# YaoChengTang/DecNet

Hardware: AMD Instinct MI355X
Metric: stereo pairs/sec at 960x540x192disp (hot path: stage-0 dense + SpaMat/SpaVar stages 1-3) (higher is better)
Workload: dtype f32 (bf16x3 on the bf16 matrix pipe); 1 GPU; BASELINE config 2: synthetic 960x540 (padded 972x540), max_disp 192->216: batch=8 synthetic pairs per GPU, feature maps of the 4-stage/scale-3 net, random-init CostRegNetNoDown(216); pairs_per_gpu=8, parallelism=dp1 (pairs sharded, all_gather of disparity maps)

## Files before the change

### decnet_amd/csrc/spamat_mfma.hip

```cpp
#include <stdlib.h>
#include <string.h>

#include "spamat_host.h"


typedef float f32x4 __attribute__((ext_vector_type(4)));
typedef int i32x4 __attribute__((ext_vector_type(4)));
typedef __bf16 bf16x8 __attribute__((ext_vector_type(8)));

namespace {

constexpr float NEG_BIG = -1.0e30f;
constexpr float LOG2E = 1.4426950408889634f;
constexpr int THREADS = 512, NWAVE = THREADS / 64;

__device__ __forceinline__ float fast_exp2(float x) { return __builtin_amdgcn_exp2f(x); }

__device__ __forceinline__ bool uniform_flag(bool f) { return __builtin_amdgcn_readfirstlane((int)f) != 0; }
template <bool SEL = true>
__device__ __forceinline__ float4 load4f(const float *__restrict__ safe, const float *__restrict__ row, int x, int W, bool ok) {
    const bool in = ok && x >= 0 && x < W;
    const float4 t = *reinterpret_cast<const float4 *>(in ? row + x : safe);
    if (!SEL) return t;
    return make_float4(in ? t.x : 0.f, in ? t.y : 0.f, in ? t.z : 0.f, in ? t.w : 0.f);
// ... 7 lines not shown
        if (x + 1 >= 0 && x + 1 < W) v.y = row[x + 1];
        if (x + 2 >= 0 && x + 2 < W) v.z = row[x + 2];
        if (x + 3 >= 0 && x + 3 < W) v.w = row[x + 3];
    }
    return v;
}
__device__ __forceinline__ float4 load4s(const float *__restrict__ row, int x, int W) {
    float4 v = make_float4(0.f, 0.f, 0.f, 0.f);
    if (x >= 0 && x < W) v.x = row[x];
    if (x + 1 >= 0 && x + 1 < W) v.y = row[x + 1];
    if (x + 2 >= 0 && x + 2 < W) v.z = row[x + 2];
    if (x + 3 >= 0 && x + 3 < W) v.w = row[x + 3];
    return v;
}

__device__ __forceinline__ int mask4_bits(const unsigned long long *__restrict__ rowbits, int x, int W) {
    if (x < 0 || x >= W) return 0;
    return (int)((rowbits[x >> 6] >> (x & 63)) & 15ull);
}

__device__ __forceinline__ int mask4_words(const unsigned *__restrict__ roww, int x, int W) {
    if (x < 0 || x >= W) return 0;
    return (int)((roww[x >> 5] >> (x & 31)) & 15u);
}

__device__ __forceinline__ void split3x8(const float (&x)[8], i32x4 &hi, i32x4 &mid, i32x4 &lo) {
    int h[8], m[8], l[8];
#pragma unroll
    for (int e = 0; e < 8; ++e) {
        h[e] = __float_as_int(x[e]) & 0xffff0000;
        const float r1 = x[e] - __int_as_float(h[e]);
        m[e] = __float_as_int(r1) & 0xffff0000;
        l[e] = __float_as_int(r1 - __int_as_float(m[e]));
    }
#pragma unroll
    for (int e = 0; e < 4; ++e) {
        hi[e] = __builtin_amdgcn_perm(h[2 * e + 1], h[2 * e], 0x07060302);
        mid[e] = __builtin_amdgcn_perm(m[2 * e + 1], m[2 * e], 0x07060302);
        lo[e] = __builtin_amdgcn_perm(l[2 * e + 1], l[2 * e], 0x07060302);
    }
}

__host__ __device__ inline int d16_pitch(int quads) { return quads + ((4 - quads) & 7); }
struct Layout {
    int SW, HALO, RP, Cq;
    int offR, offBX, offRK, offLM, offXL, offWT, total;
};
__host__ __device__ inline Layout make_layout(int C, int NT, int XT, bool d16 = false) {
    Layout l;
    l.SW = XT * 16;
    l.HALO = (NT - 1) * 16;
    l.Cq = (C + 3) & ~3;
    l.RP = ((l.HALO + l.SW + 31) & ~31) + 16;
    l.offR = 0;
    const int swh = ((XT + 1) / 2) * 16;
    const int rt = d16 ? 3 * ((C + 7) / 8) * 16 * (d16_pitch((l.HALO + swh) >> 2) + d16_pitch(swh >> 2)) : 0;
    l.offBX = l.offR + (l.Cq * l.RP > rt ? l.Cq * l.RP : rt);
    l.offRK = l.offBX + l.RP;
    l.offLM = l.offRK + l.RP + 4;
    l.offXL = l.offLM + l.SW + 16;
    l.offWT = l.offXL + l.SW;
    l.total = l.offWT + 32;
    return l;
}

__device__ __forceinline__ int wave_incl_scan(int v, int lane) {
#pragma unroll
    for (int o = 1; o < 64; o <<= 1) {
        int t = __shfl_up(v, o);
        if (lane >= o) v += t;
    }
    return v;
}

template <int M, int N, int STEP, class F>
__device__ __forceinline__ void live_tiles(int ntile, F &&f) {
    if constexpr (M < N) {
        if (STEP > 0 && M >= ntile) return;
        f(std::integral_constant<int, M>{});
        if constexpr (STEP == 2 && M + 1 < N) f(std::integral_constant<int, M + 1>{});
        live_tiles<M + (STEP > 1 ? STEP : 1), N, STEP>(ntile, f);
    }
}
template <int NTL, int MODE, int COMPACT>
__device__ __forceinline__ void softmax_passes(f32x4 (&acc)[NTL], int ntile, int D, int dl,
                                               const float *__restrict__ lds, int bias_off, int xr_off,
                                               int xlj, float mu_in,
                                               float &mx_o, float &S_o, float &mu_o, float &var_o,
                                               int m_lo = 0, int m_hi = 0) {
    constexpr int GS = COMPACT >= 2 ? 2 : COMPACT;
    int dlv = dl;
    asm volatile("" : "+v"(dlv));
    float mx0 = 0.000001f, mx1 = 0.000001f;
    (void)bias_off;
    int xo1 = xr_off;
    asm volatile("" : "+v"(xo1));
    const int *xp1 = reinterpret_cast<const int *>(lds) + xo1;
    const float xlf = (float)xlj, hD = 0.5f * (float)(D - 1), xlh = xlf - hD;
    live_tiles<0, NTL, GS>(ntile, [&](auto mc) {
        constexpr int m = decltype(mc)::value;
        {
            if (COMPACT >= 2) {
                if (COMPACT == 2 || m < m_lo || m >= m_hi) {
                    if (COMPACT == 3) asm volatile("" ::: "memory");
                    const float4 p = *reinterpret_cast<const float4 *>(xp1 + 16 * m);
                    acc[m][0] = fabsf(xlh - p.x) <= hD ? acc[m][0] : NEG_BIG;
                    acc[m][1] = fabsf(xlh - p.y) <= hD ? acc[m][1] : NEG_BIG;
                    acc[m][2] = fabsf(xlh - p.z) <= hD ? acc[m][2] : NEG_BIG;
                    acc[m][3] = fabsf(xlh - p.w) <= hD ? acc[m][3] : NEG_BIG;
                }
            } else if (COMPACT) {
                const int4 p = *reinterpret_cast<const int4 *>(xp1 + 16 * m);
                acc[m][0] = (unsigned)(xlj - p.x) < (unsigned)D ? acc[m][0] : NEG_BIG;
                acc[m][1] = (unsigned)(xlj - p.y) < (unsigned)D ? acc[m][1] : NEG_BIG;
                acc[m][2] = (unsigned)(xlj - p.z) < (unsigned)D ? acc[m][2] : NEG_BIG;
                acc[m][3] = (unsigned)(xlj - p.w) < (unsigned)D ? acc[m][3] : NEG_BIG;
            } else {
                if (m == 0 || 16 * m + 15 >= D) {
                    asm volatile("" ::: "memory");
#pragma unroll
                    for (int r = 0; r < 4; ++r) {
                        const int d = 16 * m + dlv - r;
                        acc[m][r] = (unsigned)d >= (unsigned)D ? NEG_BIG : acc[m][r];
                    }
                }
            }
            mx0 = fmaxf(fmaxf(mx0, acc[m][0]), acc[m][1]);
            mx1 = fmaxf(fmaxf(mx1, acc[m][2]), acc[m][3]);
        }
    });
    float mx = fmaxf(mx0, mx1);
    mx = fmaxf(mx, __shfl_xor(mx, 16));
    mx = fmaxf(mx, __shfl_xor(mx, 32));
    if (!COMPACT && MODE != MODE_MAT) {
        const float nmv = -mx * LOG2E;
        float Sa = 0.f, Sb = 0.f, T16a = 0.f, T16b = 0.f, Tt = 0.f;
#pragma unroll
        for (int m = 0; m < NTL; ++m) {
            if (m < ntile) {
                const float e0 = fast_exp2(fmaf(acc[m][0], LOG2E, nmv));
                const float e1 = fast_exp2(fmaf(acc[m][1], LOG2E, nmv));
                const float e2 = fast_exp2(fmaf(acc[m][2], LOG2E, nmv));
                const float e3 = fast_exp2(fmaf(acc[m][3], LOG2E, nmv));
                const float s4 = (e0 + e1) + (e2 + e3);
                const float t2 = fmaf(6.f, e3, fmaf(4.f, e2, e1 + e1));
                const float qq = fmaf(9.f, e3, fmaf(4.f, e2, e1));
                acc[m][0] = s4;
                acc[m][1] = t2;
                acc[m][2] = qq;
                if (m & 1) { Sb += s4; T16b = fmaf(s4, (float)(16 * m), T16b); }
                else { Sa += s4; T16a = fmaf(s4, (float)(16 * m), T16a); }
                Tt += t2;
            }
        }
        const float dlf = (float)dl;
        float Sl = Sa + Sb;
        float Tl = fmaf(dlf, Sl, fmaf(-0.5f, Tt, T16a + T16b));
        Sl += __shfl_xor(Sl, 16);
        Sl += __shfl_xor(Sl, 32);
        const float S = Sl + 0.000001f;
        float mu = mu_in;
        if (MODE != MODE_VAR) {
            Tl += __shfl_xor(Tl, 16);
            Tl += __shfl_xor(Tl, 32);
            mu = (Tl + 0.000001f) / S;
        }
        const float c0 = dlf - mu;
        float V0 = 0.f, V1 = 0.f;
#pragma unroll
        for (int m = 0; m < NTL; ++m) {
            if (m < ntile) {
                const float A = (float)(16 * m) + c0;
                const float u = fmaf(A, acc[m][0], -acc[m][1]);
                if (m & 1) V1 = fmaf(A, u, V1) + acc[m][2];
                else V0 = fmaf(A, u, V0) + acc[m][2];
            }
        }
        float Vl = V0 + V1;
        Vl += __shfl_xor(Vl, 16);
        Vl += __shfl_xor(Vl, 32);
        mx_o = mx; S_o = S; mu_o = mu; var_o = (Vl + 0.000001f) / S;
        return;
    }
    const float nm = -mx * LOG2E;
    float S0 = 0.f, S1 = 0.f, T0 = 0.f, T1 = 0.f;
    int xo2 = xr_off;
    asm volatile("" : "+v"(xo2));
    const int *xp2 = reinterpret_cast<const int *>(lds) + xo2;
    live_tiles<0, NTL, GS>(ntile, [&](auto mc) {
        constexpr int m = decltype(mc)::value;
        {
            int4 p;
            float4 pf;
            if (COMPACT >= 2) pf = *reinterpret_cast<const float4 *>(xp2 + 16 * m);
            else if (COMPACT) p = *reinterpret_cast<const int4 *>(xp2 + 16 * m);
#pragma unroll
            for (int r = 0; r < 4; r += 2) {
                float e0 = fast_exp2(fmaf(acc[m][r], LOG2E, nm));
                float e1 = fast_exp2(fmaf(acc[m][r + 1], LOG2E, nm));
                acc[m][r] = e0;
                acc[m][r + 1] = e1;
                S0 += e0;
                S1 += e1;
                if (MODE != MODE_VAR) {
                    if (COMPACT >= 2) {
                        T0 = fmaf(e0, xlf - (r == 0 ? pf.x : pf.z), T0);
                        T1 = fmaf(e1, xlf - (r == 0 ? pf.y : pf.w), T1);
                    } else if (COMPACT) {
                        T0 = fmaf(e0, (float)(xlj - (r == 0 ? p.x : p.z)), T0);
                        T1 = fmaf(e1, (float)(xlj - (r == 0 ? p.y : p.w)), T1);
                    } else {
                        T0 = fmaf(e0, (float)(16 * m - r), T0);
                        T1 = fmaf(e1, (float)(16 * m - r - 1), T1);
                    }
                }
            }
        }
    });
    const float dlf = (float)dl;
    float Sl = S0 + S1;
    float Tl = COMPACT ? T0 + T1 : fmaf(dlf, Sl, T0 + T1);
    Sl += __shfl_xor(Sl, 16);
    Sl += __shfl_xor(Sl, 32);
    const float S = Sl + 0.000001f;
    float mu = mu_in;
    if (MODE != MODE_VAR) {
        Tl += __shfl_xor(Tl, 16);
        Tl += __shfl_xor(Tl, 32);
        mu = (Tl + 0.000001f) / S;
    }
    float var = 0.f;
    if (MODE != MODE_MAT) {
        const float c0 = (COMPACT ? (float)xlj : dlf) - mu;
        float V0 = 0.f, V1 = 0.f;
        int xo3 = xr_off;
        asm volatile("" : "+v"(xo3));
        const int *xp3 = reinterpret_cast<const int *>(lds) + xo3;
        live_tiles<0, NTL, GS>(ntile, [&](auto mc) {
            constexpr int m = decltype(mc)::value;
            {
                int4 p;
                float4 pf;
                if (COMPACT >= 2) pf = *reinterpret_cast<const float4 *>(xp3 + 16 * m);
                else if (COMPACT) p = *reinterpret_cast<const int4 *>(xp3 + 16 * m);
#pragma unroll
                for (int r = 0; r < 4; r += 2) {
                    float d0, d1;
                    if (COMPACT >= 2) {
                        d0 = c0 - (r == 0 ? pf.x : pf.z);
                        d1 = c0 - (r == 0 ? pf.y : pf.w);
                    } else if (COMPACT) {
                        d0 = c0 - (float)(r == 0 ? p.x : p.z);
                        d1 = c0 - (float)(r == 0 ? p.y : p.w);
                    } else {
                        d0 = (float)(16 * m - r) + c0;
                        d1 = (float)(16 * m - r - 1) + c0;
                    }
                    V0 = fmaf(acc[m][r] * d0, d0, V0);
                    V1 = fmaf(acc[m][r + 1] * d1, d1, V1);
                }
            }
        });
        float Vl = V0 + V1;
        Vl += __shfl_xor(Vl, 16);
        Vl += __shfl_xor(Vl, 32);
        var = (Vl + 0.000001f) / S;
    }
    mx_o = mx; S_o = S; mu_o = mu; var_o = var;
}


__device__ __forceinline__ void dense16_loads8(float4 (&v)[8], const float *__restrict__ src, size_t plane, int g, int C,
                                               int x, int W, bool al) {
    if (al) {
        const bool whole = x + 3 < W;
#pragma unroll
        for (int c = 0; c < 8; ++c)
            v[c] = load4f<false>(src, src + (size_t)(8 * g + c) * plane, x, W, whole && 8 * g + c < C);
        __builtin_amdgcn_sched_barrier(0);
        if (__ballot(x < 0) != 0ull) {
#pragma unroll
            for (int c = 0; c < 8; ++c)
                if (x < 0) v[c] = make_float4(0.f, 0.f, 0.f, 0.f);
        }
        if (C & 7) {
#pragma unroll
            for (int c = 0; c < 8; ++c) {
                const bool ch = 8 * g + c < C;
                v[c] = make_float4(ch ? v[c].x : 0.f, ch ? v[c].y : 0.f, ch ? v[c].z : 0.f, ch ? v[c].w : 0.f);
            }
        }
        if ((W & 3) && x < W && !whole) {
#pragma unroll
            for (int c = 0; c < 8; ++c)
                v[c] = 8 * g + c < C ? load4s(src + (size_t)(8 * g + c) * plane, x, W) : make_float4(0.f, 0.f, 0.f, 0.f);
        }
    } else {
#pragma unroll
        for (int c = 0; c < 8; ++c)
            v[c] = 8 * g + c < C ? load4s(src + (size_t)(8 * g + c) * plane, x, W) : make_float4(0.f, 0.f, 0.f, 0.f);
    }
}

__device__ __forceinline__ void dense16_item_loads(float4 (&v)[8], int it, const float *__restrict__ lrow,
                                                   const float *__restrict__ rrow, size_t plane, int C, int W, int xs,
                                                   int SW, int HALO, int nRw) {
    const bool al = uniform_flag(((((uintptr_t)rrow) | ((uintptr_t)lrow) | ((uintptr_t)(plane * 4))) & 15) == 0);
    const int cg_n = (C + 7) >> 3, nqR = nRw >> 2, nqL = SW >> 2;
    const int nR_items = cg_n * nqR;
    const bool isL = it >= nR_items;
    const int k = isL ? it - nR_items : it, nq = isL ? nqL : nqR;
    const int g = k / nq, jq = k - g * nq;
    const float *src = isL ? lrow : rrow;
    const int x = isL ? xs + 4 * jq : xs - HALO + 4 * jq;
    dense16_loads8(v, src, plane, g, C, x, W, al);
}

template <int NT, int MODE, int CGT, bool PRE = false>
__device__ __forceinline__ void dense16_body(int *RT, const float *BX, const float *LM, const float *smem,
                                             const float *__restrict__ lrow, const float *__restrict__ rrow,
                                             const float *__restrict__ disparity, float *__restrict__ out,
                                             float *__restrict__ var_out, float *__restrict__ sum_sim,
                                             float *__restrict__ max_cost, size_t plane, size_t rowpix, int C, int W,
                                             int D, int xs, int XT, int SW, int HALO, int nRw, const float4 *pre = nullptr) {
    const int tid = threadIdx.x, lane = tid & 63, wave = tid >> 6;
    struct { int CG; } lo = {(C + 7) >> 3};
    const int PR = d16_pitch(nRw >> 2), PL = d16_pitch(SW >> 2);
    int *LT = RT + 3 * lo.CG * 16 * PR;
    {
        const bool al = uniform_flag(((((uintptr_t)rrow) | ((uintptr_t)lrow) | ((uintptr_t)(plane * 4))) & 15) == 0);
        const int cg_n = lo.CG, nqR = nRw >> 2, nqL = SW >> 2;
        const int nR_items = cg_n * nqR, n_items = nR_items + cg_n * nqL;
#pragma unroll 1
        for (int it = tid; it < n_items; it += THREADS) {
            const bool isL = it >= nR_items;
            const int k = isL ? it - nR_items : it, nq = isL ? nqL : nqR;
            const int g = k / nq, jq = k - g * nq;
            const float *src = isL ? lrow : rrow;
            const int x = isL ? xs + 4 * jq : xs - HALO + 4 * jq;
            float4 v[8];
            if (PRE && it == tid) {
#pragma unroll
                for (int c = 0; c < 8; ++c) v[c] = pre[c];
            } else {
                dense16_loads8(v, src, plane, g, C, x, W, al);
            }
            const int P = isL ? PL : PR;
            int *dst = (isL ? LT : RT) + (g * 4 * P + jq) * 4;
            const int tstride = cg_n * 16 * P;
#pragma unroll
            for (int pz = 0; pz < 4; ++pz) {
                float xv[8];
#pragma unroll
                for (int c = 0; c < 8; ++c) xv[c] = pz == 0 ? v[c].x : pz == 1 ? v[c].y : pz == 2 ? v[c].z : v[c].w;
                i32x4 th, tm, tl;
                split3x8(xv, th, tm, tl);
                *reinterpret_cast<i32x4 *>(dst + pz * 4 * P) = th;
                *reinterpret_cast<i32x4 *>(dst + tstride + pz * 4 * P) = tm;
                *reinterpret_cast<i32x4 *>(dst + 2 * tstride + pz * 4 * P) = tl;
            }
        }
    }
    __syncthreads();

    const int j = lane & 15, q = lane >> 4;
    const int dl = j - 4 * q;
    constexpr int CGB = CGT ? CGT : 1;
    const int cg_n = CGT ? CGT : lo.CG;
    const int tA_big = q >> 1, tA_small = q == 0 ? 0 : q == 2 ? 1 : 2;
    const int tB_big = q & 1, tB_small = q == 1 ? 0 : q == 3 ? 1 : 2;
    const int gsR = 16 * PR, gsL = 16 * PL;
    for (int xt = wave; xt < XT; xt += NWAVE) {
        const int x0 = xs + xt * 16;
        if (x0 >= W) break;
        const int x = x0 + j;
        const size_t pix = rowpix + x;
        const bool inside = x < W;
        const float rm = LM[xt * 16 + j];
        if (__ballot(rm != 0.f) == 0ull) {
            if (inside && q == 0) {
                if (MODE != MODE_VAR) out[pix] = 0.f;
                if (MODE != MODE_MAT) var_out[pix] = 0.f;
                sum_sim[pix] = 0.f;
                max_cost[pix] = 0.f;
            }
            continue;
        }
        f32x4 acc[NT];
#pragma unroll
        for (int m = 0; m < NT; ++m) {
            const float4 bz = *reinterpret_cast<const float4 *>(BX + (HALO + xt * 16) + 4 * q - 16 * m);
            acc[m] = f32x4{bz.x, bz.y, bz.z, bz.w};
        }
        const int sa = (j & 3) * PR + 4 * xt + (j >> 2), sb = (j & 3) * PL + 4 * xt + (j >> 2);
        const int *a_small = RT + (tA_small * cg_n * 4 * PR + sa) * 4;
        const int *a_big = RT + (tA_big * cg_n * 4 * PR + sa) * 4;
        const int *b_small = LT + (tB_small * cg_n * 4 * PL + sb) * 4;
        const int *b_big = LT + (tB_big * cg_n * 4 * PL + sb) * 4;
#pragma unroll
        for (int g = 0; g < CGB; ++g) {
            for (int gg = g; gg < cg_n; gg += CGB) {
                const i32x4 bs = *reinterpret_cast<const i32x4 *>(b_small + gg * gsL);
                const i32x4 bb = *reinterpret_cast<const i32x4 *>(b_big + gg * gsL);
#pragma unroll
                for (int m = 0; m < NT; ++m) {
                    const i32x4 av = *reinterpret_cast<const i32x4 *>(a_small + gg * gsR + (NT - 1 - m) * 16);
                    acc[m] = __builtin_amdgcn_mfma_f32_16x16x32_bf16(__builtin_bit_cast(bf16x8, av),
                                                                     __builtin_bit_cast(bf16x8, bs), acc[m], 0, 0, 0);
                }
#pragma unroll
                for (int m = 0; m < NT; ++m) {
                    const i32x4 av = *reinterpret_cast<const i32x4 *>(a_big + gg * gsR + (NT - 1 - m) * 16);
                    acc[m] = __builtin_amdgcn_mfma_f32_16x16x32_bf16(__builtin_bit_cast(bf16x8, av),
                                                                     __builtin_bit_cast(bf16x8, bb), acc[m], 0, 0, 0);
                }
            }
        }
        float mx, S, mu, var;
        const float mu_in = (MODE == MODE_VAR && inside) ? disparity[pix] : 0.f;
        softmax_passes<NT, MODE, 0>(acc, NT, D, dl, smem, 0, 0, 0, mu_in, mx, S, mu, var);
        if (inside && q == 0) {
            const bool on = rm != 0.f;
            if (MODE != MODE_VAR) out[pix] = on ? mu : 0.f;
            if (MODE != MODE_MAT) var_out[pix] = on ? var : 0.f;
            sum_sim[pix] = on ? S : 0.f;
            max_cost[pix] = on ? mx : 0.f;
        }
    }

}

template <int NT, int MODE, int KQ, int PPT, int NTHR, int CAP, int NTCMAX>
__device__ __forceinline__ int sparse_row_body(
    const float *__restrict__ ref, const float *__restrict__ tar, const float *__restrict__ rmask,
    const float *__restrict__ tmask, const float *__restrict__ disparity, float *__restrict__ out,
    float *__restrict__ var_out, float *__restrict__ sum_sim, float *__restrict__ max_cost, int C,
    int H, int W, int D, int row, int dense_pct, int mbits, int *fr_out = nullptr, int *fl_out = nullptr);
constexpr int MID_CAP = 640;

template <int NT, int MODE, int KQ, bool D16>
__device__ __forceinline__ void spamat_fwd_segment(
    const float *__restrict__ ref, const float *__restrict__ tar, const float *__restrict__ rmask,
    const float *__restrict__ tmask, const float *__restrict__ disparity, float *__restrict__ out,
    float *__restrict__ var_out, float *__restrict__ sum_sim, float *__restrict__ max_cost, int C,
    int H, int W, int D, int XT, int allow_compact, int marker, int seg, int row, int compact_pct, int mbits) {
    const float mark = marker ? sum_sim[(size_t)row * W + (size_t)seg * (XT * 16)] : -1.0f;
    if (marker && !(mark < 0.f))
        return;
    if constexpr (KQ == 2) {
        if (marker == 2 && mark == -2.0f) {
            if (sparse_row_body<NT, MODE, KQ, 4, THREADS, MID_CAP, NT + 1>(ref, tar, rmask, tmask, disparity, out, var_out,
                                                                          sum_sim, max_cost, C, H, W, D, row, 100,
                                                                          mbits) == 1)
                return;
            __syncthreads();
        }
    }
    extern __shared__ __attribute__((aligned(16))) float smem[];
    const Layout lo = make_layout(C, NT, XT, D16);
    float *Rs = smem + lo.offR;
    float *BX = smem + lo.offBX;
    int *XR = reinterpret_cast<int *>(BX);
    int *RK = reinterpret_cast<int *>(smem + lo.offRK);
    float *LM = smem + lo.offLM;
    int *RKL = reinterpret_cast<int *>(LM);
    int *XL = reinterpret_cast<int *>(smem + lo.offXL);
    int *WT = reinterpret_cast<int *>(smem + lo.offWT);
    const int SW = lo.SW, HALO = lo.HALO, RP = lo.RP;
    const int kq_n = KQ ? KQ : lo.Cq / 4;
    constexpr int KB = KQ ? KQ : 1;

    const int tid = threadIdx.x, lane = tid & 63, wave = tid >> 6;
    const int b = row / H, y = row - b * H;
    const int xs = seg * SW;
    const int nRw = HALO + SW;
    const size_t plane = (size_t)H * W;
    const float *lrow = ref + ((size_t)b * C * H + y) * W;
    const float *rrow = tar + ((size_t)b * C * H + y) * W;
    const float *trow = tmask + (size_t)row * W;
    const float *mrow = rmask + (size_t)row * W;
    const size_t rowpix = (size_t)row * W;
    const unsigned long long *tbits = reinterpret_cast<const unsigned long long *>(tmask) + (size_t)row * ((W + 63) >> 6);
    const unsigned long long *lbits = reinterpret_cast<const unsigned long long *>(rmask) + (size_t)row * ((W + 63) >> 6);

    unsigned mf_wr = 0, mf_wl = 0;
    if constexpr (D16) {
        if (mbits == 2) {
            const int q4 = tid * 4, xr_ = xs - HALO + q4, xl_ = xs + q4;
            const unsigned *hw = reinterpret_cast<const unsigned *>(max_cost + rowpix);
            mf_wr = hw[(q4 < nRw && xr_ >= 0 && xr_ < W) ? xr_ >> 5 : 0];
            mf_wl = hw[((W + 31) >> 5) + ((q4 < SW && xl_ < W) ? xl_ >> 5 : 0)];
        }
    }
    float4 d16_pre[D16 ? 8 : 1];
    if constexpr (D16) {
        const int xta = (XT + 1) / 2;
        const int n_items = ((C + 7) >> 3) * (((HALO + xta * 16) >> 2) + ((xta * 16) >> 2));
        if (tid < n_items) dense16_item_loads(d16_pre, tid, lrow, rrow, plane, C, W, xs, xta * 16, HALO, HALO + xta * 16);
    }
    const bool al_r = ((((uintptr_t)rrow) | ((uintptr_t)(plane * 4))) & 15) == 0;
    const int st_nq = nRw >> 2;
    const int st_rpp = THREADS / st_nq;
    const int st_r0 = tid / st_nq, st_jq = tid - st_r0 * st_nq;
    float4 st_v[D16 ? 1 : 8];
    float bfirst[(!D16 && KQ > 0) ? KQ : 1];
    if constexpr (!D16) {
        if (st_r0 < st_rpp) {
            const int x = xs - HALO + 4 * st_jq;
#pragma unroll
            for (int u = 0; u < 8; ++u) {
                const int c = st_r0 + u * st_rpp;
                st_v[u] = c < C ? load4_lanes(rrow + (size_t)c * plane, x, W, al_r) : make_float4(0.f, 0.f, 0.f, 0.f);
            }
        }
        if constexpr (KQ > 0) {
            const int jl = lane & 15, ql = lane >> 4;
            const int x = xs + wave * 16 + jl;
            const bool ok = wave < XT && x < W;
#pragma unroll
            for (int s = 0; s < KQ; ++s) bfirst[s] = (ok && 4 * s + ql < C) ? lrow[(size_t)(4 * s + ql) * plane + x] : 0.f;
        }
    }

    const int p4 = tid * 4;
    int fr = 0, fl = 0;
    {
        const bool alm = (((uintptr_t)trow) & 15) == 0 && (((uintptr_t)mrow) & 15) == 0;
        const bool almu = D16 && uniform_flag(alm && (W & 3) == 0);
        if (p4 < nRw) {
            const int x = xs - HALO + p4;
            if (mbits == 2) {
                if (D16) fr = (x >= 0 && x < W) ? (int)((mf_wr >> (x & 31)) & 15u) : 0;
                else fr = mask4_words(reinterpret_cast<const unsigned *>(max_cost + rowpix), x, W);
            } else if (mbits) {
                fr = mask4_bits(tbits, x, W);
            } else {
                float4 tv = almu ? load4f(trow, trow, x, W, true) : load4_lanes(trow, x, W, alm);
                fr = (tv.x != 0.f) | ((tv.y != 0.f) << 1) | ((tv.z != 0.f) << 2) | ((tv.w != 0.f) << 3);
            }
            float4 bv4;
            bv4.x = (fr & 1) ? 0.f : NEG_BIG;
            bv4.y = (fr & 2) ? 0.f : NEG_BIG;
            bv4.z = (fr & 4) ? 0.f : NEG_BIG;
            bv4.w = (fr & 8) ? 0.f : NEG_BIG;
            *reinterpret_cast<float4 *>(BX + p4) = bv4;
        }
        if (p4 < SW) {
            float4 mv;
            if (mbits) {
                if (D16 && mbits == 2) fl = (xs + p4 < W) ? (int)((mf_wl >> ((xs + p4) & 31)) & 15u) : 0;
                else fl = mbits == 2 ? mask4_words(reinterpret_cast<const unsigned *>(max_cost + rowpix) + ((W + 31) >> 5), xs + p4, W)
                                : mask4_bits(lbits, xs + p4, W);
                mv = make_float4((fl & 1) ? 1.f : 0.f, (fl & 2) ? 1.f : 0.f, (fl & 4) ? 1.f : 0.f, (fl & 8) ? 1.f : 0.f);
            } else {
                mv = almu ? load4f(mrow, mrow, xs + p4, W, true) : load4_lanes(mrow, xs + p4, W, alm);
                fl = (mv.x != 0.f) | ((mv.y != 0.f) << 1) | ((mv.z != 0.f) << 2) | ((mv.w != 0.f) << 3);
            }
            *reinterpret_cast<float4 *>(LM + p4) = mv;
        }
    }
    {
        const int ir = wave_incl_scan(__popc(fr), lane), il = wave_incl_scan(__popc(fl), lane);
        if (lane == 63) { WT[wave] = ir; WT[8 + wave] = il; }
    }

    int nR = 0, nL = 0;
    bool compact = false;
    if constexpr (D16) {
        __syncthreads();
#pragma unroll
        for (int w = 0; w < NWAVE; ++w) { nR += WT[w]; nL += WT[8 + w]; }
        const int validL = min(SW, W - xs);
        const int validR = min(W, xs + SW) - max(0, xs - HALO);
        compact = allow_compact && ((long)nL * nR * 100 < (long)validL * validR * compact_pct);
        if (!compact) {
            const int xta = (XT + 1) / 2, xtb = XT - xta;
            dense16_body<NT, MODE, (KQ + 1) / 2, true>(reinterpret_cast<int *>(Rs), BX, LM, smem, lrow, rrow, disparity, out,
                                                       var_out, sum_sim, max_cost, plane, rowpix, C, W, D, xs, xta, xta * 16,
                                                       HALO, HALO + xta * 16, d16_pre);
            if (xtb > 0 && xs + xta * 16 < W) {
                __syncthreads();
                dense16_body<NT, MODE, (KQ + 1) / 2>(reinterpret_cast<int *>(Rs), BX + xta * 16, LM + xta * 16, smem, lrow,
                                                     rrow, disparity, out, var_out, sum_sim, max_cost, plane, rowpix, C,
                                                     W, D, xs + xta * 16, xtb, xtb * 16, HALO, HALO + xtb * 16);
            }
            return;
        }
    }
    {
        const bool al = al_r;
        const int rpp = st_rpp;
        const int r0 = st_r0, jq = st_jq;
        if (r0 < rpp) {
            const int jj = 4 * jq, x = xs - HALO + jj;
            for (int c0 = r0; c0 < lo.Cq; c0 += 8 * rpp) {
                float4 v[8];
                if (!D16 && c0 == r0) {
#pragma unroll
                    for (int u = 0; u < 8; ++u) v[u] = st_v[D16 ? 0 : u];
                } else {
#pragma unroll
                    for (int u = 0; u < 8; ++u) {
                        const int c = c0 + u * rpp;
                        v[u] = c < C ? load4_lanes(rrow + (size_t)c * plane, x, W, al) : make_float4(0.f, 0.f, 0.f, 0.f);
                    }
                }
#pragma unroll
                for (int u = 0; u < 8; ++u) {
                    const int c = c0 + u * rpp;
                    if (c < lo.Cq) *reinterpret_cast<float4 *>(Rs + c * RP + jj) = v[u];
                }
            }
        }
        for (int c = tid; c < lo.Cq; c += THREADS) Rs[c * RP + RP - 1] = 0.f;
    }
    __syncthreads();

    const int validL = min(SW, W - xs);
    const int validR = min(W, xs + SW) - max(0, xs - HALO);
    if constexpr (!D16) {
#pragma unroll
        for (int w = 0; w < NWAVE; ++w) { nR += WT[w]; nL += WT[8 + w]; }
        compact = allow_compact && ((long)nL * nR * 100 < (long)validL * validR * compact_pct);
    }

    const int j = lane & 15, q = lane >> 4;

    if constexpr (!D16) if (!compact) {
        const int dl = j - 4 * q;
        float bv[KQ <= 6 ? KB : 1], bcur[KB];
        float rm = 0.f;
        auto fetch_left = [&](int xt, float (&dst)[KB]) {
            const int x = xs + xt * 16 + j;
            const bool ok = xt < XT && x < W;
            if (KQ) {
#pragma unroll
                for (int s = 0; s < KQ; ++s)
                    dst[s] = (ok && 4 * s + q < C) ? lrow[(size_t)(4 * s + q) * plane + x] : 0.f;
            }
        };
        constexpr bool PREF = KQ <= 6;
        if constexpr (PREF && KQ > 0) {
#pragma unroll
            for (int s = 0; s < KB; ++s) bv[s] = bfirst[s];
        } else if constexpr (PREF) {
            fetch_left(wave, bv);
        }
        for (int xt = wave; xt < XT; xt += NWAVE) {
            const int x0 = xs + xt * 16;
            if (x0 >= W) break;
            const int x = x0 + j;
            const size_t pix = rowpix + x;
            const bool inside = x < W;
            rm = LM[xt * 16 + j];
            if constexpr (PREF) {
#pragma unroll
                for (int s = 0; s < KB; ++s) bcur[s] = bv[s];
                fetch_left(xt + NWAVE, bv);
            } else if (KQ > 0 && xt == wave) {
#pragma unroll
                for (int s = 0; s < KB; ++s) bcur[s] = bfirst[KQ > 0 ? s : 0];
            } else {
// ... 87 lines not shown
    while (S > 16 && (long)S * nL > 24L * validL) S >>= 1;
    __syncthreads();
    constexpr int NTC = NT + 1;
    while (S > 16) {
        int bad = 0;
        for (int g = tid; g * S < SW; g += THREADS) {
            const int jlo = max(0, g * S + HALO - (D - 1)), jhi = min(nRw - 1, g * S + HALO + S - 1);
            if (RK[jhi + 1] - RK[jlo] > 16 * NTC - 15) bad = 1;
        }
        if (!__syncthreads_or(bad)) break;
        S >>= 1;
    }

    for (int p = tid; p < validL; p += THREADS) {
        if (RKL[p + 1] == RKL[p]) {
            const size_t pix = rowpix + xs + p;
            if (MODE != MODE_VAR) out[pix] = 0.f;
            if (MODE != MODE_MAT) var_out[pix] = 0.f;
            sum_sim[pix] = 0.f;
            max_cost[pix] = 0.f;
        }
    }

    const int ngroups = (SW + S - 1) / S;
    for (int g = wave; g < ngroups; g += NWAVE) {
        const int gx = g * S;
        const int e0 = __builtin_amdgcn_readfirstlane(RKL[gx]), e1 = __builtin_amdgcn_readfirstlane(RKL[min(gx + S, SW)]);
        if (e1 == e0) continue;
        const int jlo = max(0, gx + HALO - (D - 1)), jhi = min(nRw - 1, gx + HALO + S - 1);
        const int r_lo = __builtin_amdgcn_readfirstlane(RK[jlo]), r_hi = __builtin_amdgcn_readfirstlane(RK[jhi + 1]);
        const int t0 = r_lo >> 4;
        const int ntile = r_hi > r_lo ? ((r_hi - 1) >> 4) - t0 + 1 : 0;
        for (int e = e0; e < e1; e += 16) {
            const bool act = e + j < e1;
            const int xl = XL[act ? e + j : e1 - 1];
            const int x = xs + xl;
            const size_t pix = rowpix + x;
            float bcur[KB];
            if (KQ) {
#pragma unroll
                for (int s = 0; s < KQ; ++s)
                    bcur[s] = (act && 4 * s + q < C) ? lrow[(size_t)(4 * s + q) * plane + x] : 0.f;
            }
            f32x4 acc[NTC];
            const int *xa = XR + 16 * t0 + j;
            live_tiles<0, NTC, 1>(ntile, [&](auto mc) {
                constexpr int m = decltype(mc)::value;
                {
                    const float *ap = Rs + q * RP + xa[16 * m];
                    f32x4 a4 = f32x4{0.f, 0.f, 0.f, 0.f};
                    if (KQ) {
#pragma unroll
                        for (int s = 0; s < KQ; ++s)
                            a4 = __builtin_amdgcn_mfma_f32_16x16x4f32(ap[4 * s * RP], bcur[s], a4, 0, 0, 0);
                    } else {
                        const float *bp = lrow + (size_t)q * plane + x;
                        for (int s = 0; s < kq_n; ++s) {
                            const float lv = (act && 4 * s + q < C) ? bp[(size_t)4 * s * plane] : 0.f;
                            a4 = __builtin_amdgcn_mfma_f32_16x16x4f32(ap[4 * s * RP], lv, a4, 0, 0, 0);
                        }
                    }
                    acc[m] = a4;
                }
            });
            float mx, Ssum, mu, var;
            const float mu_in = (MODE == MODE_VAR && act) ? disparity[pix] : 0.f;
            softmax_passes<NTC, MODE, 1>(acc, ntile, D, 0, smem, 0, lo.offBX + 16 * t0 + 4 * q, xl + HALO, mu_in,
                                         mx, Ssum, mu, var);
            if (act && q == 0) {
                if (MODE != MODE_VAR) out[pix] = mu;
                if (MODE != MODE_MAT) var_out[pix] = var;
                sum_sim[pix] = Ssum;
                max_cost[pix] = mx;
            }
        }
    }
}

template <int NT, int MODE, int KQ, bool D16>
__global__ __launch_bounds__(THREADS, (KQ > 6 ? 2 : 4)) void spamat_fwd_mfma(
    const float *__restrict__ ref, const float *__restrict__ tar, const float *__restrict__ rmask,
    const float *__restrict__ tmask, const float *__restrict__ disparity, float *__restrict__ out,
    float *__restrict__ var_out, float *__restrict__ sum_sim, float *__restrict__ max_cost, int C,
    int H, int W, int D, int segs_per_row, int XT, int allow_compact, int marker, int compact_pct, int mbits) {
    spamat_fwd_segment<NT, MODE, KQ, D16>(ref, tar, rmask, tmask, disparity, out, var_out, sum_sim, max_cost, C, H, W,
                                          D, XT, allow_compact, marker, blockIdx.x % segs_per_row,
                                          blockIdx.x / segs_per_row, compact_pct, mbits);
}

constexpr int SP_THREADS = 256, SP_CAP = 256;
constexpr size_t sparse_row_words(int kq, int ppt, int nthr, int cap) {
    return (size_t)(cap + 32) + 2 * (size_t)(nthr * ppt / 2 + 2) + cap + 32 + 2 * (size_t)4 * kq * (cap + 16);
}

template <int NT, int MODE, int KQ, int PPT, int NTHR, int CAP, int NTCMAX>
__device__ __forceinline__ int sparse_row_body(
    const float *__restrict__ ref, const float *__restrict__ tar, const float *__restrict__ rmask,
    const float *__restrict__ tmask, const float *__restrict__ disparity, float *__restrict__ out,
    float *__restrict__ var_out, float *__restrict__ sum_sim, float *__restrict__ max_cost, int C,
    int H, int W, int D, int row, int dense_pct, int mbits, int *fr_out, int *fl_out) {
    constexpr int CQ = 4 * KQ, NTC = NT + 1 < NTCMAX ? NT + 1 : NTCMAX;
    constexpr int SP_NWAVE_ = NTHR / 64, SP_FP_ = CAP + 16;
    extern __shared__ __attribute__((aligned(16))) float smem[];
    constexpr int NPX = NTHR * PPT, RKW = NPX / 2 + 2;
    constexpr int offXR = 0, offRK = CAP + 32, offRKL = offRK + RKW, offXL = offRKL + RKW,
                  offWT = offXL + CAP, offRF = offWT + 32, offLF = offRF + CQ * SP_FP_;
    float *XR = smem + offXR;
    unsigned short *RK = reinterpret_cast<unsigned short *>(smem + offRK);
    unsigned short *RKL = reinterpret_cast<unsigned short *>(smem + offRKL);
    int *XL = reinterpret_cast<int *>(smem) + offXL;
    int *WT = reinterpret_cast<int *>(smem) + offWT;
    float *RF = smem + offRF, *LF = smem + offLF;

    const int tid = threadIdx.x, lane = tid & 63, wave = tid >> 6;
    const int b = row / H, y = row - b * H;
    const size_t plane = (size_t)H * W, rowpix = (size_t)row * W;
    const float *lrow = ref + ((size_t)b * C * H + y) * W;
    const float *rrow = tar + ((size_t)b * C * H + y) * W;
    const float *trow = tmask + rowpix, *mrow = rmask + rowpix;

    constexpr bool ALL = CAP > 256 && PPT == 4;
    const int p4 = tid * PPT;
    float4 lv[ALL ? CQ : 1], rv[ALL ? CQ : 1];
    if constexpr (ALL) {
        const bool alf = ((W & 3) == 0) && ((((uintptr_t)lrow) | ((uintptr_t)rrow) | ((uintptr_t)(plane * 4))) & 15) == 0;
#pragma unroll
        for (int c = 0; c < CQ; ++c) {
            const bool ok = p4 < W && c < C;
            lv[c] = ok ? load4_lanes(lrow + (size_t)c * plane, p4, W, alf) : make_float4(0.f, 0.f, 0.f, 0.f);
            rv[c] = ok ? load4_lanes(rrow + (size_t)c * plane, p4, W, alf) : make_float4(0.f, 0.f, 0.f, 0.f);
        }
    }
    int fr = 0, fl = 0;
    {
        const bool alm = ((W & 3) == 0) && ((((uintptr_t)trow) | ((uintptr_t)mrow)) & 15) == 0;
#pragma unroll
        for (int u = 0; u < PPT; u += 4) {
            if (p4 + u < W) {
                if (mbits == 2) {
                    const unsigned *hw = reinterpret_cast<const unsigned *>(max_cost + rowpix);
                    fr |= mask4_words(hw, p4 + u, W) << u;
                    fl |= mask4_words(hw + ((W + 31) >> 5), p4 + u, W) << u;
                } else if (mbits) {
                    const int wpr = (W + 63) >> 6;
                    fr |= mask4_bits(reinterpret_cast<const unsigned long long *>(tmask) + (size_t)row * wpr, p4 + u, W) << u;
                    fl |= mask4_bits(reinterpret_cast<const unsigned long long *>(rmask) + (size_t)row * wpr, p4 + u, W) << u;
                } else {
                    const float4 tv = load4_lanes(trow, p4 + u, W, alm), mv = load4_lanes(mrow, p4 + u, W, alm);
                    fr |= ((tv.x != 0.f) | ((tv.y != 0.f) << 1) | ((tv.z != 0.f) << 2) | ((tv.w != 0.f) << 3)) << u;
                    fl |= ((mv.x != 0.f) | ((mv.y != 0.f) << 1) | ((mv.z != 0.f) << 2) | ((mv.w != 0.f) << 3)) << u;
                }
            }
        }
    }
    if (fr_out) { *fr_out = fr; *fl_out = fl; }
    const int cr = __popc(fr), cl = __popc(fl);
    const int ir = wave_incl_scan(cr, lane), il = wave_incl_scan(cl, lane);
    if (lane == 63) { WT[wave] = ir; WT[8 + wave] = il; }
    __syncthreads();
    int nR = 0, nL = 0, baseR = 0, baseL = 0;
#pragma unroll
    for (int w = 0; w < SP_NWAVE_; ++w) {
        if (w < wave) { baseR += WT[w]; baseL += WT[8 + w]; }
        nR += WT[w];
        nL += WT[8 + w];
    }
    nR = __builtin_amdgcn_readfirstlane(nR);
    nL = __builtin_amdgcn_readfirstlane(nL);
    if ((long)nL * nR * 100 >= (long)W * W * dense_pct) return 0;
    if (nL > CAP || nR > CAP) return (nL <= MID_CAP && nR <= MID_CAP) ? 2 : 0;
// ... 137 lines not shown
                if (MODE != MODE_VAR) *reinterpret_cast<float4 *>(out + pix) = make_float4(r[0][0], r[0][1], r[0][2], r[0][3]);
                if (MODE != MODE_MAT) *reinterpret_cast<float4 *>(var_out + pix) = make_float4(r[1][0], r[1][1], r[1][2], r[1][3]);
                *reinterpret_cast<float4 *>(sum_sim + pix) = make_float4(r[2][0], r[2][1], r[2][2], r[2][3]);
                *reinterpret_cast<float4 *>(max_cost + pix) = make_float4(r[3][0], r[3][1], r[3][2], r[3][3]);
            } else {
#pragma unroll
                for (int k = 0; k < 4; ++k) {
                    if (p4 + u + k < W) {
                        if (MODE != MODE_VAR) out[pix + k] = r[0][k];
                        if (MODE != MODE_MAT) var_out[pix + k] = r[1][k];
                        sum_sim[pix + k] = r[2][k];
                        max_cost[pix + k] = r[3][k];
                    }
                }
            }
        }
    }
    return 1;
}

template <int NT, int MODE, int KQ, int PPT>
__global__ __launch_bounds__(SP_THREADS, PPT == 4 ? 6 : 5) void spamat_fwd_sparse(
    const float *__restrict__ ref, const float *__restrict__ tar, const float *__restrict__ rmask,
    const float *__restrict__ tmask, const float *__restrict__ disparity, float *__restrict__ out,
    float *__restrict__ var_out, float *__restrict__ sum_sim, float *__restrict__ max_cost, int C,
    int H, int W, int D, int seg_w, int dense_pct, int mbits, int handover) {
    const int row = blockIdx.x;
    int fr = 0, fl = 0;
    const int rc = sparse_row_body<NT, MODE, KQ, PPT, SP_THREADS, SP_CAP, 8>(ref, tar, rmask, tmask, disparity, out, var_out,
                                                                            sum_sim, max_cost, C, H, W, D, row, dense_pct, mbits,
                                                                            &fr, &fl);
    if (rc != 1) {
        const size_t rowpix = (size_t)row * W;
        const float mark = rc == 2 ? -2.0f : -1.0f;
        for (int x = threadIdx.x * seg_w; x < W; x += SP_THREADS * seg_w) sum_sim[rowpix + x] = mark;
        if (handover) {
            extern __shared__ __attribute__((aligned(16))) float smem[];
            unsigned *wb = reinterpret_cast<unsigned *>(smem);
            const int nw = (W + 31) >> 5, p4 = threadIdx.x * PPT;
            __syncthreads();
            for (int i = threadIdx.x; i < 2 * nw; i += SP_THREADS) wb[i] = 0u;
            __syncthreads();
            if (p4 < W) {
                if (fr) atomicOr(&wb[p4 >> 5], (unsigned)fr << (p4 & 31));
                if (fl) atomicOr(&wb[nw + (p4 >> 5)], (unsigned)fl << (p4 & 31));
            }
            __syncthreads();
            for (int i = threadIdx.x; i < 2 * nw; i += SP_THREADS) reinterpret_cast<unsigned *>(max_cost + rowpix)[i] = wb[i];
        }
    }
}

template <int NT, int KQ>
int launch_nt(const SpaFwd &a) {
    const int B = a.B, C = a.C, H = a.H, W = a.W, D = a.D, allow_compact = a.allow_compact, mbits = a.mbits;
    const int xt_row = ceil_div(W, 16);
    static const int dense_fp32 = [] { const char *e = getenv("DECNET_SPAMAT_DENSE"); return e && !strcmp(e, "fp32"); }();
    const bool d16 = KQ == 2 && !dense_fp32;
    auto bytes = [&](int xt) { return (size_t)4 * make_layout(C, NT, xt, d16).total; };
    const size_t budget2 = (DECNET_LDS_BYTES - 2048) / 2, budget1 = DECNET_LDS_BYTES - 1024;
    int XT = xt_row > 64 ? ceil_div(xt_row, ceil_div(xt_row, 64)) : xt_row;
    if (bytes(XT) > budget2) {
        int segs = ceil_div(xt_row, XT) + 1;
        while (segs < xt_row && bytes(ceil_div(xt_row, segs)) > budget2) ++segs;
        int xt2 = ceil_div(xt_row, segs);
        if (bytes(xt2) <= budget2) XT = xt2;
        else {
            while (XT > 1 && bytes(XT) > budget1) --XT;
        }
    }
    XT = (XT + 1) & ~1;
    if (XT > 64) XT = 64;
    const size_t lds = bytes(XT);
    if (lds > budget1 || make_layout(C, NT, XT, d16).RP > 2048) return DECNET_ERR_UNSUPPORTED;
    const int segs = ceil_div(xt_row, XT);
    dim3 block(THREADS);
    constexpr int compact_pct = 35;
    constexpr int sparse_pct = 45;
    dim3 grid((unsigned)((size_t)B * H * segs));
    int marker = allow_compact && KQ == 2 && W <= 2048;
    static const bool mid_off = [] { const char *e = getenv("DECNET_SPAMAT_MID"); return e && atoi(e) == 0; }();
    size_t lds_launch = lds;
    static const bool handover_off = [] { const char *e = getenv("DECNET_SPAMAT_HANDOVER"); return e && atoi(e) == 0; }();
    const int handover = (KQ > 0 && KQ <= 6 && marker && segs == 1 && !mbits && 2 * ((W + 31) / 32) <= W && !handover_off) ? 1 : 0;
    if (KQ == 2 && marker && segs == 1 && !mid_off) {
        const size_t need = 4 * sparse_row_words(KQ, 4, THREADS, MID_CAP);
        if (need <= budget2 + 8192) {
            marker = 2;
            if (need > lds_launch) lds_launch = need;
        }
    }
    if constexpr (KQ > 0 && KQ <= 6) if (marker) {
        const int ppt = W <= 1024 ? 4 : 8;
        const size_t slds = 4 * sparse_row_words(KQ, ppt, SP_THREADS, SP_CAP);
        int rc = spamat_with_mode(a.mode, [&](auto M) {
            return spamat_with_flag(ppt == 4, [&](auto P4) {
                return decnet_launch(spamat_fwd_sparse<NT, M(), KQ, (P4() ? 4 : 8)>, dim3((unsigned)(B * H)), dim3(SP_THREADS),
                                     slds, a.stream, a.ref, a.tar, a.rmask, a.tmask, a.disparity, a.out, a.var_out, a.sum_sim,
                                     a.max_cost, C, H, W, D, XT * 16, sparse_pct, mbits, handover);
            });
        });
        if (rc) return rc;
    }
    auto band = [&](auto M, auto D16) {
        return decnet_launch(spamat_fwd_mfma<NT, M(), KQ, D16()>, grid, block, lds_launch, a.stream, a.ref, a.tar, a.rmask,
                             a.tmask, a.disparity, a.out, a.var_out, a.sum_sim, a.max_cost, C, H, W, D, segs, XT,
                             allow_compact, marker, compact_pct, handover ? 2 : mbits);
    };
    return spamat_with_mode(a.mode, [&](auto M) {
        if constexpr (KQ == 2) return spamat_with_flag(d16, [&](auto D16) { return band(M, D16); });
        else return band(M, std::false_type{});
    });
}

template <int NT>
int launch_kq(const SpaFwd &a) {
    const int C = a.C;
    if (C <= 8 && C > 4) return launch_nt<NT, 2>(a);
    if (C <= 24 && C > 20) return launch_nt<NT, 6>(a);
    if (C <= 72 && C > 68) return launch_nt<NT, 18>(a);
    return launch_nt<NT, 0>(a);
}

}

int decnet_mfma_forward(const SpaFwd &a) {
    const int D = a.D;
    const int need = D <= 1 ? 1 : (D - 1 + 15) / 16 + 1;
    if (need <= 3) return launch_kq<3>(a);
    if (need <= 6) return launch_kq<6>(a);
    if (need <= 8) return launch_kq<8>(a);
    if (need <= 11) return launch_kq<11>(a);
    if (need <= 15) return launch_kq<15>(a);
    if (need <= 18) return launch_kq<18>(a);
    return DECNET_ERR_UNSUPPORTED;
}
```

Before: 5093 pairs/s.

## Skip dead disparity tiles for left-edge pixel tiles in dense16 SpaMat path

For pixel tiles near the left image border, disparity tiles beyond x are entirely invalid. The change runs MFMA accumulation, bias init and the softmax moment passes only over the live disparity tiles there. It also skips loading right-image halo items at negative x. Left-edge tiles are paired (first with last) across waves to balance their uneven work. This adds template instantiations and an env knob that restores the full-tile behaviour, and it relies on the skipped tiles having no effect on the softmax result.

```diff
diff --git a/decnet_amd/csrc/spamat_mfma.hip b/decnet_amd/csrc/spamat_mfma.hip
--- a/decnet_amd/csrc/spamat_mfma.hip
+++ b/decnet_amd/csrc/spamat_mfma.hip
@@ -113,13 +113,13 @@
         live_tiles<M + (STEP > 1 ? STEP : 1), N, STEP>(ntile, f);
     }
 }
-template <int NTL, int MODE, int COMPACT>
+template <int NTL, int MODE, int COMPACT, int GATE = -1>
 __device__ __forceinline__ void softmax_passes(f32x4 (&acc)[NTL], int ntile, int D, int dl,
                                                const float *__restrict__ lds, int bias_off, int xr_off,
                                                int xlj, float mu_in,
                                                float &mx_o, float &S_o, float &mu_o, float &var_o,
                                                int m_lo = 0, int m_hi = 0) {
-    constexpr int GS = COMPACT >= 2 ? 2 : COMPACT;
+    constexpr int GS = GATE >= 0 ? GATE : COMPACT >= 2 ? 2 : COMPACT;
     int dlv = dl;
     asm volatile("" : "+v"(dlv));
     float mx0 = 0.000001f, mx1 = 0.000001f;
@@ -166,24 +166,34 @@
     if (!COMPACT && MODE != MODE_MAT) {
         const float nmv = -mx * LOG2E;
         float Sa = 0.f, Sb = 0.f, T16a = 0.f, T16b = 0.f, Tt = 0.f;
-#pragma unroll
-        for (int m = 0; m < NTL; ++m) {
-            if (m < ntile) {
-                const float e0 = fast_exp2(fmaf(acc[m][0], LOG2E, nmv));
-                const float e1 = fast_exp2(fmaf(acc[m][1], LOG2E, nmv));
-                const float e2 = fast_exp2(fmaf(acc[m][2], LOG2E, nmv));
-                const float e3 = fast_exp2(fmaf(acc[m][3], LOG2E, nmv));
-                const float s4 = (e0 + e1) + (e2 + e3);
-                const float t2 = fmaf(6.f, e3, fmaf(4.f, e2, e1 + e1));
-                const float qq = fmaf(9.f, e3, fmaf(4.f, e2, e1));
-                acc[m][0] = s4;
-                acc[m][1] = t2;
-                acc[m][2] = qq;
-                if (m & 1) { Sb += s4; T16b = fmaf(s4, (float)(16 * m), T16b); }
-                else { Sa += s4; T16a = fmaf(s4, (float)(16 * m), T16a); }
-                Tt += t2;
-            }
-        }
+#define DECNET_MOMENTS_TILE(m)                                                                         \
+    {                                                                                                  \
+        const float e0 = fast_exp2(fmaf(acc[m][0], LOG2E, nmv));                                       \
+        const float e1 = fast_exp2(fmaf(acc[m][1], LOG2E, nmv));                                       \
+        const float e2 = fast_exp2(fmaf(acc[m][2], LOG2E, nmv));                                       \
+        const float e3 = fast_exp2(fmaf(acc[m][3], LOG2E, nmv));                                       \
+        const float s4 = (e0 + e1) + (e2 + e3);                                                        \
+        const float t2 = fmaf(6.f, e3, fmaf(4.f, e2, e1 + e1));                                        \
+        const float qq = fmaf(9.f, e3, fmaf(4.f, e2, e1));                                             \
+        acc[m][0] = s4;                                                                                \
+        acc[m][1] = t2;                                                                                \
+        acc[m][2] = qq;                                                                                \
+        if (m & 1) { Sb += s4; T16b = fmaf(s4, (float)(16 * m), T16b); }                               \
+        else { Sa += s4; T16a = fmaf(s4, (float)(16 * m), T16a); }                                     \
+        Tt += t2;                                                                                      \
+    }
+        if constexpr (GS > 0) {
+            live_tiles<0, NTL, GS>(ntile, [&](auto mc) {
+                constexpr int m = decltype(mc)::value;
+                DECNET_MOMENTS_TILE(m)
+            });
+        } else {
+#pragma unroll
+            for (int m = 0; m < NTL; ++m) {
+                if (m < ntile) DECNET_MOMENTS_TILE(m)
+            }
+        }
+#undef DECNET_MOMENTS_TILE
         const float dlf = (float)dl;
         float Sl = Sa + Sb;
         float Tl = fmaf(dlf, Sl, fmaf(-0.5f, Tt, T16a + T16b));
@@ -198,15 +208,25 @@
         }
         const float c0 = dlf - mu;
         float V0 = 0.f, V1 = 0.f;
-#pragma unroll
-        for (int m = 0; m < NTL; ++m) {
-            if (m < ntile) {
-                const float A = (float)(16 * m) + c0;
-                const float u = fmaf(A, acc[m][0], -acc[m][1]);
-                if (m & 1) V1 = fmaf(A, u, V1) + acc[m][2];
-                else V0 = fmaf(A, u, V0) + acc[m][2];
-            }
-        }
+#define DECNET_CENTRAL_TILE(m)                                                                         \
+    {                                                                                                  \
+        const float A = (float)(16 * m) + c0;                                                          \
+        const float u = fmaf(A, acc[m][0], -acc[m][1]);                                                \
+        if (m & 1) V1 = fmaf(A, u, V1) + acc[m][2];                                                    \
+        else V0 = fmaf(A, u, V0) + acc[m][2];                                                          \
+    }
+        if constexpr (GS > 0) {
+            live_tiles<0, NTL, GS>(ntile, [&](auto mc) {
+                constexpr int m = decltype(mc)::value;
+                DECNET_CENTRAL_TILE(m)
+            });
+        } else {
+#pragma unroll
+            for (int m = 0; m < NTL; ++m) {
+                if (m < ntile) DECNET_CENTRAL_TILE(m)
+            }
+        }
+#undef DECNET_CENTRAL_TILE
         float Vl = V0 + V1;
         Vl += __shfl_xor(Vl, 16);
         Vl += __shfl_xor(Vl, 32);
@@ -335,7 +355,7 @@
 
 __device__ __forceinline__ void dense16_item_loads(float4 (&v)[8], int it, const float *__restrict__ lrow,
                                                    const float *__restrict__ rrow, size_t plane, int C, int W, int xs,
-                                                   int SW, int HALO, int nRw) {
+                                                   int SW, int HALO, int nRw, bool left_skip) {
     const bool al = uniform_flag(((((uintptr_t)rrow) | ((uintptr_t)lrow) | ((uintptr_t)(plane * 4))) & 15) == 0);
     const int cg_n = (C + 7) >> 3, nqR = nRw >> 2, nqL = SW >> 2;
     const int nR_items = cg_n * nqR;
@@ -344,6 +364,7 @@
     const int g = k / nq, jq = k - g * nq;
     const float *src = isL ? lrow : rrow;
     const int x = isL ? xs + 4 * jq : xs - HALO + 4 * jq;
+    if (left_skip && !isL && x < 0) return;
     dense16_loads8(v, src, plane, g, C, x, W, al);
 }
 
@@ -353,7 +374,9 @@
                                              const float *__restrict__ disparity, float *__restrict__ out,
                                              float *__restrict__ var_out, float *__restrict__ sum_sim,
                                              float *__restrict__ max_cost, size_t plane, size_t rowpix, int C, int W,
-                                             int D, int xs, int XT, int SW, int HALO, int nRw, const float4 *pre = nullptr) {
+                                             int D, int xs, int XT, int SW, int HALO, int nRw, const float4 *pre = nullptr,
+                                             bool left_skip_arg = false) {
+    const bool left_skip = PRE && left_skip_arg;
     const int tid = threadIdx.x, lane = tid & 63, wave = tid >> 6;
     struct { int CG; } lo = {(C + 7) >> 3};
     const int PR = d16_pitch(nRw >> 2), PL = d16_pitch(SW >> 2);
@@ -369,6 +392,7 @@
             const int g = k / nq, jq = k - g * nq;
             const float *src = isL ? lrow : rrow;
             const int x = isL ? xs + 4 * jq : xs - HALO + 4 * jq;
+            if (left_skip && !isL && x < 0) continue;
             float4 v[8];
             if (PRE && it == tid) {
 #pragma unroll
@@ -401,9 +425,9 @@
     const int tA_big = q >> 1, tA_small = q == 0 ? 0 : q == 2 ? 1 : 2;
     const int tB_big = q & 1, tB_small = q == 1 ? 0 : q == 3 ? 1 : 2;
     const int gsR = 16 * PR, gsL = 16 * PL;
-    for (int xt = wave; xt < XT; xt += NWAVE) {
+    auto wave_tile = [&](int xt, auto edge, int live) __attribute__((always_inline)) {
+        constexpr int GS = decltype(edge)::value ? 1 : 0;
         const int x0 = xs + xt * 16;
-        if (x0 >= W) break;
         const int x = x0 + j;
         const size_t pix = rowpix + x;
         const bool inside = x < W;
@@ -415,14 +439,14 @@
                 sum_sim[pix] = 0.f;
                 max_cost[pix] = 0.f;
             }
-            continue;
+            return;
         }
         f32x4 acc[NT];
-#pragma unroll
-        for (int m = 0; m < NT; ++m) {
+        live_tiles<0, NT, GS>(live, [&](auto mc) {
+            constexpr int m = decltype(mc)::value;
             const float4 bz = *reinterpret_cast<const float4 *>(BX + (HALO + xt * 16) + 4 * q - 16 * m);
             acc[m] = f32x4{bz.x, bz.y, bz.z, bz.w};
-        }
+        });
         const int sa = (j & 3) * PR + 4 * xt + (j >> 2), sb = (j & 3) * PL + 4 * xt + (j >> 2);
         const int *a_small = RT + (tA_small * cg_n * 4 * PR + sa) * 4;
         const int *a_big = RT + (tA_big * cg_n * 4 * PR + sa) * 4;
@@ -433,23 +457,23 @@
             for (int gg = g; gg < cg_n; gg += CGB) {
                 const i32x4 bs = *reinterpret_cast<const i32x4 *>(b_small + gg * gsL);
                 const i32x4 bb = *reinterpret_cast<const i32x4 *>(b_big + gg * gsL);
-#pragma unroll
-                for (int m = 0; m < NT; ++m) {
+                live_tiles<0, NT, GS>(live, [&](auto mc) {
+                    constexpr int m = decltype(mc)::value;
                     const i32x4 av = *reinterpret_cast<const i32x4 *>(a_small + gg * gsR + (NT - 1 - m) * 16);
                     acc[m] = __builtin_amdgcn_mfma_f32_16x16x32_bf16(__builtin_bit_cast(bf16x8, av),
                                                                      __builtin_bit_cast(bf16x8, bs), acc[m], 0, 0, 0);
-                }
-#pragma unroll
-                for (int m = 0; m < NT; ++m) {
+                });
+                live_tiles<0, NT, GS>(live, [&](auto mc) {
+                    constexpr int m = decltype(mc)::value;
                     const i32x4 av = *reinterpret_cast<const i32x4 *>(a_big + gg * gsR + (NT - 1 - m) * 16);
                     acc[m] = __builtin_amdgcn_mfma_f32_16x16x32_bf16(__builtin_bit_cast(bf16x8, av),
                                                                      __builtin_bit_cast(bf16x8, bb), acc[m], 0, 0, 0);
-                }
+                });
             }
         }
         float mx, S, mu, var;
         const float mu_in = (MODE == MODE_VAR && inside) ? disparity[pix] : 0.f;
-        softmax_passes<NT, MODE, 0>(acc, NT, D, dl, smem, 0, 0, 0, mu_in, mx, S, mu, var);
+        softmax_passes<NT, MODE, 0, GS>(acc, live, D, dl, smem, 0, 0, 0, mu_in, mx, S, mu, var);
         if (inside && q == 0) {
             const bool on = rm != 0.f;
             if (MODE != MODE_VAR) out[pix] = on ? mu : 0.f;
@@ -457,8 +481,21 @@
             sum_sim[pix] = on ? S : 0.f;
             max_cost[pix] = on ? mx : 0.f;
         }
-    }
-
+    };
+    const int NE = left_skip ? min(XT, max(0, NT - 1 - xs / 16)) : 0;
+    const int npair = (NE + 1) >> 1;
+    int item = wave;
+    if constexpr (PRE) {
+        for (; item < npair; item += NWAVE) {
+            const int iu = __builtin_amdgcn_readfirstlane(item);
+#pragma unroll 1
+            for (int xt = iu;; xt = NE - 1 - iu) {
+                if (xs + xt * 16 < W) wave_tile(xt, std::true_type{}, xs / 16 + xt + 1);
+                if (xt >= NE - 1 - iu) break;
+            }
+        }
+    }
+    for (int xt = NE + item - npair; xt < XT && xs + xt * 16 < W; xt += NWAVE) wave_tile(xt, std::false_type{}, NT);
 }
 
 template <int NT, int MODE, int KQ, int PPT, int NTHR, int CAP, int NTCMAX>
@@ -474,7 +511,7 @@
     const float *__restrict__ ref, const float *__restrict__ tar, const float *__restrict__ rmask,
     const float *__restrict__ tmask, const float *__restrict__ disparity, float *__restrict__ out,
     float *__restrict__ var_out, float *__restrict__ sum_sim, float *__restrict__ max_cost, int C,
-    int H, int W, int D, int XT, int allow_compact, int marker, int seg, int row, int compact_pct, int mbits) {
+    int H, int W, int D, int XT, int allow_compact, int marker, int seg, int row, int compact_pct, int mbits, int left_all) {
     const float mark = marker ? sum_sim[(size_t)row * W + (size_t)seg * (XT * 16)] : -1.0f;
     if (marker && !(mark < 0.f))
         return;
@@ -527,7 +564,7 @@
     if constexpr (D16) {
         const int xta = (XT + 1) / 2;
         const int n_items = ((C + 7) >> 3) * (((HALO + xta * 16) >> 2) + ((xta * 16) >> 2));
-        if (tid < n_items) dense16_item_loads(d16_pre, tid, lrow, rrow, plane, C, W, xs, xta * 16, HALO, HALO + xta * 16);
+        if (tid < n_items) dense16_item_loads(d16_pre, tid, lrow, rrow, plane, C, W, xs, xta * 16, HALO, HALO + xta * 16, !left_all);
     }
     const bool al_r = ((((uintptr_t)rrow) | ((uintptr_t)(plane * 4))) & 15) == 0;
     const int st_nq = nRw >> 2;
@@ -608,7 +645,7 @@
             const int xta = (XT + 1) / 2, xtb = XT - xta;
             dense16_body<NT, MODE, (KQ + 1) / 2, true>(reinterpret_cast<int *>(Rs), BX, LM, smem, lrow, rrow, disparity, out,
                                                        var_out, sum_sim, max_cost, plane, rowpix, C, W, D, xs, xta, xta * 16,
-                                                       HALO, HALO + xta * 16, d16_pre);
+                                                       HALO, HALO + xta * 16, d16_pre, !left_all);
             if (xtb > 0 && xs + xta * 16 < W) {
                 __syncthreads();
                 dense16_body<NT, MODE, (KQ + 1) / 2>(reinterpret_cast<int *>(Rs), BX + xta * 16, LM + xta * 16, smem, lrow,
@@ -862,10 +899,10 @@
     const float *__restrict__ ref, const float *__restrict__ tar, const float *__restrict__ rmask,
     const float *__restrict__ tmask, const float *__restrict__ disparity, float *__restrict__ out,
     float *__restrict__ var_out, float *__restrict__ sum_sim, float *__restrict__ max_cost, int C,
-    int H, int W, int D, int segs_per_row, int XT, int allow_compact, int marker, int compact_pct, int mbits) {
+    int H, int W, int D, int segs_per_row, int XT, int allow_compact, int marker, int compact_pct, int mbits, int left_all) {
     spamat_fwd_segment<NT, MODE, KQ, D16>(ref, tar, rmask, tmask, disparity, out, var_out, sum_sim, max_cost, C, H, W,
                                           D, XT, allow_compact, marker, blockIdx.x % segs_per_row,
-                                          blockIdx.x / segs_per_row, compact_pct, mbits);
+                                          blockIdx.x / segs_per_row, compact_pct, mbits, left_all);
 }
 
 constexpr int SP_THREADS = 256, SP_CAP = 256;
@@ -1169,6 +1206,7 @@
     static const bool mid_off = [] { const char *e = getenv("DECNET_SPAMAT_MID"); return e && atoi(e) == 0; }();
     size_t lds_launch = lds;
     static const bool handover_off = [] { const char *e = getenv("DECNET_SPAMAT_HANDOVER"); return e && atoi(e) == 0; }();
+    static const int left_all = [] { const char *e = getenv("DECNET_SPAMAT_LEFT_TILES"); return e && !strcmp(e, "all"); }();
     const int handover = (KQ > 0 && KQ <= 6 && marker && segs == 1 && !mbits && 2 * ((W + 31) / 32) <= W && !handover_off) ? 1 : 0;
     if (KQ == 2 && marker && segs == 1 && !mid_off) {
         const size_t need = 4 * sparse_row_words(KQ, 4, THREADS, MID_CAP);
@@ -1192,7 +1230,7 @@
     auto band = [&](auto M, auto D16) {
         return decnet_launch(spamat_fwd_mfma<NT, M(), KQ, D16()>, grid, block, lds_launch, a.stream, a.ref, a.tar, a.rmask,
                              a.tmask, a.disparity, a.out, a.var_out, a.sum_sim, a.max_cost, C, H, W, D, segs, XT,
-                             allow_compact, marker, compact_pct, handover ? 2 : mbits);
+                             allow_compact, marker, compact_pct, handover ? 2 : mbits, left_all);
     };
     return spamat_with_mode(a.mode, [&](auto M) {
         if constexpr (KQ == 2) return spamat_with_flag(d16, [&](auto D16) { return band(M, D16); });
```

After: 5116 pairs/s (median of 6 runs). No clear change (+0.5%).
